# cschin/Peregrine

Hardware: AMD Instinct MI355X
Metric: confirmed overlaps/sec (ovlp_t records, index+overlap stages, seqdb resident in HBM) (higher is better)
Workload: dtype u8/u32 integer

## Files before the change

### peregrine_amd/csrc/pgx_replay.h

```cpp
#pragma once
#include "pgx_internal.h"

namespace pgx {
namespace rp {

constexpr uint32_t NIL = 0;
constexpr uint32_t NONE = 0xFFFFFFFFu;
constexpr int END_FUZZ = 48;
enum { T_OVERLAP = 0, T_CONTAINS = 1, T_CONTAINED = 2 };

constexpr uint32_t NIN = 58;
struct alignas(16) PHot {
  unsigned long long key;
  uint32_t own;
  uint32_t pad;
};
struct alignas(256) PCold {
  uint32_t cnt;
  uint32_t rhead;
  uint32_t in[NIN];
  uint32_t pad[4];
};
static_assert(sizeof(PHot) == 16 && sizeof(PCold) == 256, "pair slot = 16 hot bytes + four cold cache lines");
struct MSlot {
  unsigned long long a;
  uint32_t b;
  uint32_t req;
};
struct Item {
  uint32_t pslot;
  uint32_t info;
  uint32_t mslot;
  uint32_t next;
};
struct RNode {
  uint32_t next, bucket;
};
constexpr uint32_t I_GUESS = 1u << 18, I_UNFILED = 1u << 19;
#ifndef PGX_SPARSE_CAP
#define PGX_SPARSE_CAP 65536
#endif
constexpr uint32_t SPARSE_CAP = PGX_SPARSE_CAP;
constexpr uint32_t LIST_CAP = 262144;
constexpr uint32_t DEV_LIST = 0xFFFFFFFFu, DEV_LIST_WIN = 0xFFFFFFFEu;
enum : uint32_t { OV_ITEMS = 1, OV_NODES = 2, OV_REQS = 4, OV_PAIRS = 8, OV_MEMO = 16, OV_QOFF = 32, OV_PASSES = 64 };
constexpr uint8_t F_DUP = 1, F_GUESS = 2, F_UNFILED = 4;
constexpr uint8_t F_BIG = 8;

struct alignas(64) Counters {
  uint32_t item_top, rnode_top, nreq, overflow;
  uint32_t pad0[12];
  uint32_t ndirty, min_dirty, max_dirty, pad;
  uint32_t nbig;
  uint32_t nbig_total;
  uint32_t pad1[10];
  unsigned long long lookups, skips, evals, records;
#ifdef PGX_BIG_STATS
  uint32_t big_max_steps, big_long, big_long_n, big_evals;
  unsigned long long big_pairs, pad2[1];
#else
  unsigned long long pad2[4];
#endif
};

struct R {
  uint32_t nb;
  const uint32_t *bid, *bstart;
  const uint64_t *y0;
  const uint8_t *dir;
  const uint32_t *rlen;
  PHot *ph;
  PCold *pc;
  uint32_t cshift;
  uint32_t pmask;
  MSlot *mt;
  uint32_t mmask;
  Item *items;
  uint32_t item_cap;
  RNode *rn;
  uint32_t rn_cap;
  pgx_align_key *rq_key;
  pgx_match *rq_res;
  uint32_t req_cap, settled;
  uint32_t memo_used;
  uint8_t *dirty, *evaluated, *parity, *bflags, *ever;
  uint32_t *ihead, *inum, *ohead, *lookups, *skips;
  uint32_t *dlist;
  uint32_t *blist;
  uint32_t wlist0;
  uint4 *wcur;
  Counters *c;
  unsigned long long *spread;
// ... 113 lines not shown
  const uint32_t *w = reinterpret_cast<const uint32_t *>(&r.pc[slot >> r.cshift]);
  const uint4 h1 = *reinterpret_cast<const uint4 *>(w);
  const uint32_t c = min(h1.x, NIN);
  if (c > 0 && h1.z > j + 1 && h1.z <= r.nb) r.dirty[h1.z - 1] = 1;
  if (c > 1 && h1.w > j + 1 && h1.w <= r.nb) r.dirty[h1.w - 1] = 1;
  for (uint32_t q = 2; q < c; q += 8) {
    const uint4 a = *reinterpret_cast<const uint4 *>(w + 2 + q), b = *reinterpret_cast<const uint4 *>(w + 6 + q);
    const uint32_t x[8] = {a.x, a.y, a.z, a.w, b.x, b.y, b.z, b.w};
#pragma unroll
    for (uint32_t k = 0; k < 8; ++k)
      if (q + k < c && x[k] > j + 1 && x[k] <= r.nb) r.dirty[x[k] - 1] = 1;
  }
  if (c < NIN) return;
  for (uint32_t nd = h1.y; nd != NIL; nd = r.rn[nd - 1].next) {
    const uint32_t rb = r.rn[nd - 1].bucket;
    if (rb > j) r.dirty[rb] = 1;
  }
}

struct M128 {
  uint64_t lo, hi;
};
__device__ __forceinline__ int popc128(M128 m) { return __popcll(m.lo) + __popcll(m.hi); }
__device__ __forceinline__ bool any128(M128 m) { return (m.lo | m.hi) != 0; }
__device__ __forceinline__ int ctz128(M128 m) { return m.lo ? __builtin_ctzll(m.lo) : 64 + __builtin_ctzll(m.hi); }
__device__ __forceinline__ int nth128(M128 m, uint32_t nth) {
  const uint32_t cl = (uint32_t)__popcll(m.lo);
  uint64_t w = m.lo;
  int base = 0;
  if (nth > cl) w = m.hi, nth -= cl, base = 64;
  for (uint32_t k = 1; k < nth; ++k) w &= w - 1;
  return base + __builtin_ctzll(w);
}
__device__ __forceinline__ M128 upto128(int stop) {
  M128 m;
  m.lo = stop >= 63 ? ~0ULL : ((2ULL << stop) - 1ULL);
  m.hi = stop < 64 ? 0ULL : (stop >= 127 ? ~0ULL : ((2ULL << (stop - 64)) - 1ULL));
  return m;
}
__device__ __forceinline__ M128 and128(M128 a, M128 b) { return M128{a.lo & b.lo, a.hi & b.hi}; }
__device__ __forceinline__ M128 andn128(M128 a, M128 b) { return M128{a.lo & ~b.lo, a.hi & ~b.hi}; }
__device__ __forceinline__ M128 shr128(M128 m, uint32_t s) {
  if (s >= 128) return M128{0, 0};
  if (s >= 64) return M128{m.hi >> (s - 64), 0};
  if (s == 0) return m;
  return M128{m.lo >> s | m.hi << (64 - s), m.hi >> s};
}
__device__ __forceinline__ M128 shl128(M128 m, uint32_t s) {
  if (s >= 128) return M128{0, 0};
  if (s >= 64) return M128{0, m.lo << (s - 64)};
  if (s == 0) return m;
  return M128{m.lo << s, m.hi << s | m.lo >> (64 - s)};
}
__device__ __forceinline__ M128 or128(M128 a, M128 b) { return M128{a.lo | b.lo, a.hi | b.hi}; }




constexpr int LOOK_NB = 4;
constexpr uint8_t FACT_VALID = 1, FACT_PRESENT = 2, FACT_ACCEPTED = 4, FACT_GUESSED = 8, FACT_UNFILED = 16;
constexpr int FACT_TYPE_SHIFT = 5;
#ifndef PGX_BIG_NW
#define PGX_BIG_NW 8
#endif
constexpr int BIG_NW = PGX_BIG_NW;
constexpr int BIG_NR = BIG_NW / 2;
constexpr uint32_t BIG_WG = 512;
constexpr uint32_t SET_CAP = 2048, CLAIM_CAP = 1024;
constexpr uint32_t CB = 4096;

__global__ void k_setup(R r, uint32_t *hist);
__global__ void k_init_slots(uint4 *__restrict__ wcur, uint32_t nslots, uint32_t n_dense, uint32_t wlist0, Counters *c);
__global__ void k_eval(R r, uint32_t lo, uint32_t hi, uint32_t nlist);
template <int GLT, int PW>
__global__ void k_eval_rows(R r, uint32_t lo, uint32_t hi, uint32_t nlist);
__global__ void k_eval_big(R r, uint32_t lo, uint32_t hi, uint32_t nlist);
__global__ void k_update(R r, uint32_t lo, uint32_t hi, uint32_t nlist);
__global__ void k_count_a(R r, uint32_t rlo, uint32_t rhi, uint32_t *__restrict__ blk);
__global__ void k_count_b(R r, uint32_t rlo, uint32_t rhi, const uint32_t *__restrict__ blk, uint32_t nblk);
__global__ void k_file(R r, uint32_t limit);
__global__ void k_settle(R r);
__global__ void k_emit(R r, const uint32_t *__restrict__ off, pgx_ovlp *__restrict__ out);
__global__ void k_count_pairs(const PHot *__restrict__ ph, uint32_t cap, unsigned long long *__restrict__ out);

}
}
```

### peregrine_amd/csrc/pgx_replay.hip

```cpp
#include <optional>

#include "pgx_replay.h"

namespace pgx {
using namespace rp;
namespace {
uint32_t pow2_at_least(size_t x) {
  size_t c = 1024;
  while (c < x) c <<= 1;
  return (uint32_t)c;
}
unsigned cdiv256(size_t n) { return (unsigned)((n + 255) / 256); }
int env_int(const char *name, int unset) { return getenv(name) ? atoi(getenv(name)) : unset; }
template <typename T>
void alloc_tagged(const char *tag, DevBuf<T> &buf, size_t n) { MemTag t(tag); buf.alloc(n); }

constexpr size_t ITEMS_PER_ENTRY = 6, ITEMS_PER_BUCKET = 64, NODES_PER_ENTRY = 8, REQS_PER_ENTRY = 1;
constexpr size_t STATE_PER_BUCKET = 64;
constexpr double TABLE_LOAD = 0.4;

struct Usage {
  double pairs = 0, reqs = 0, items = 0, nodes = 0;
  void raise(const Usage &u) { pairs = std::max(pairs, u.pairs), reqs = std::max(reqs, u.reqs), items = std::max(items, u.items), nodes = std::max(nodes, u.nodes); }
};
// ... 199 lines not shown
    if (r.big_min || r.dup_min) {
      fetch(false);
      use_big = hc->nbig_total != 0;
    }
    cblk.alloc((nb + CB - 1) / CB * 3);
  }
  void setup_with_histogram() {
    DevBuf<uint32_t> hist(32);
    PGX_HIP(hipMemsetAsync(hist.p, 0, 32 * sizeof(uint32_t), s));
    hipLaunchKernelGGL(k_setup, dim3(cdiv256(nb)), dim3(256), 0, s, r, hist.p);
    uint32_t h[32];
    hist.download(h, 32);
    sync();
    fprintf(stderr, "[pgx]   buckets by entries / 8 (last class: >= 120):");
    for (int i = 0; i < 16; ++i) fprintf(stderr, " %u", h[i]);
    fprintf(stderr, "\n[pgx]   ... of those holding a read twice (one partner at a time):");
    for (int i = 0; i < 16; ++i) fprintf(stderr, " %u", h[16 + i]);
    fprintf(stderr, "\n");
  }
  void fetch(bool totals, bool counters = true) {
    if (counters) PGX_HIP(hipMemcpyAsync(hc, dc.p, sizeof(Counters), hipMemcpyDeviceToHost, s));
    if (totals) PGX_HIP(hipMemcpyAsync(rs.hs, spread.p, SPREAD * 8 * sizeof(unsigned long long), hipMemcpyDeviceToHost, s));
    sync();
    if (totals) sum_totals();
  }
  void sum_totals() {
    const unsigned long long *hs = rs.hs;
    hc->evals = hc->lookups = hc->skips = 0;
    hc->records = 0;
    for (uint32_t i = 0; i < SPREAD; ++i) hc->evals += hs[i * 8], hc->lookups += hs[i * 8 + 1], hc->skips += hs[i * 8 + 2], hc->records += hs[i * 8 + 7];
#ifdef PGX_BIG_STATS
    unsigned long long b3 = 0, b4 = 0, b5 = 0, b6 = 0, b7 = 0;
    for (uint32_t i = 0; i < SPREAD; ++i) b3 += hs[i * 8 + 3], b4 += hs[i * 8 + 4], b5 += hs[i * 8 + 5], b6 += hs[i * 8 + 6], b7 += hs[i * 8 + 7];
    fprintf(stderr, "[pgx]   k_eval_big so far: %u evaluations, %llu steps, %llu rows committed; steps cut at a duplicate %llu, ended by a containment %llu, all rows %llu; longest %u steps, %u evaluations of >= 64 steps (entries %u); %llu pairs looked up\n",
            hc->big_evals, b3, b4, b5, b6, b7, hc->big_max_steps, hc->big_long, hc->big_long_n, hc->big_pairs);
#endif
#ifdef PGX_SETTLE_STATS
    unsigned long long c3 = 0, c4 = 0, c5 = 0, c6 = 0;
    for (uint32_t i = 0; i < SPREAD; ++i) c3 += hs[i * 8 + 3], c4 += hs[i * 8 + 4], c5 += hs[i * 8 + 5], c6 += hs[i * 8 + 6];
    fprintf(stderr, "[pgx]   wrong guesses so far: type %llu, rejected short overlap %llu, rejected no match %llu, rejected other %llu\n", c3, c4, c5, c6);
#endif
  }
  void learn_dirty() { n_dirty = hc->ndirty, known = true, d_lo = n_dirty ? hc->min_dirty : 0, d_hi = n_dirty ? hc->max_dirty + 1 : 0; }
  uint32_t gave_up(uint32_t ov) {
    if (trace || !(ov & (OV_ITEMS | OV_NODES | OV_REQS | OV_PAIRS | OV_MEMO)))
      fprintf(stderr, "[pgx] note: the device replay gave up (code %u: items %u of %u, reader nodes %u of %u, requests %u of %u)\n", ov,
              hc->item_top, r.item_cap, hc->rnode_top, r.rn_cap, hc->nreq, r.req_cap);
    return ov;
  }
  void count(uint32_t lo = 0, uint32_t hi = NONE) {
    hi = std::min<uint32_t>(hi, (uint32_t)nb);
    const uint32_t nbl = std::max<uint32_t>(1, (hi - lo + CB - 1) / CB);
    std::optional<KernelTimer> tm;
    if (timed) tm.emplace("replay_misc", 0);
    hipLaunchKernelGGL(k_count_a, dim3(nbl), dim3(256), 0, s, r, lo, hi, cblk.p);
    hipLaunchKernelGGL(k_count_b, dim3(nbl), dim3(256), 0, s, r, lo, hi, cblk.p, nbl);
  }
  void count_all() { count(), have_list = true; }
  void pass(uint32_t lo, uint32_t hi, uint32_t list, Narrow narrow, uint32_t groups, uint64_t units) {
    std::optional<KernelTimer> tm;
    if (timed) tm.emplace(narrow == Narrow::rows ? "replay_rows" : "replay_dense", units);
    const bool walled = deep && list != DEV_LIST;
    double td = 0, t_eval = 0;
    if (walled) sync(), td = wall_ms();
    if (list == DEV_LIST_WIN) count(lo, hi);
    const uint32_t a = list ? 0u : lo, b = list ? (uint32_t)nb : hi;
    const uint32_t big_a = list == DEV_LIST_WIN ? LIST_CAP : list == DEV_LIST ? groups : lo;
    const dim3 big_grid(std::min<uint32_t>(BIG_WG, groups)), big_block(64 * BIG_NW), grid(cdiv256((size_t)groups * GL));
// ... 266 lines not shown
```

### peregrine_amd/csrc/pgx_replay_eval.hip

```cpp
#include "pgx_replay.h"

namespace pgx {
namespace rp {

__global__ __launch_bounds__(256) void k_eval(R r, uint32_t lo, uint32_t hi, uint32_t nlist) {
  __shared__ uint32_t s_rid[GPB][128], s_pos[GPB][128], s_rl[GPB][128];
  __shared__ uint8_t s_dir[GPB][128];
  const int lane = threadIdx.x & 63, gl = lane & (GL - 1), gbase = lane & ~(GL - 1), gib = threadIdx.x / GL;
  const uint32_t wave = (blockIdx.x * blockDim.x + threadIdx.x) >> 6;
  const uint64_t jj = bucket_of_group(r, lo, hi, nlist, wave * GPW + (uint32_t)(lane / GL));
  const uint32_t j = (uint32_t)jj;
  bool alive = jj < hi && r.dirty[j] && !r.c->overflow;
  if (alive && (r.bflags[j] & F_BIG)) {
    if (gl == 0) {
      const uint32_t at = atomicAdd(&r.c->nbig, 1u);
      if (at < LIST_CAP) r.blist[at] = j;
    }
    alive = false;
  }
  {
    const uint64_t am = __ballot(alive);
    if (!am) return;
    if (lane == (int)__builtin_ctzll(am)) atomicAdd(&r.spread[(wave % SPREAD) * 8], (unsigned long long)(__popcll(am) / GL));
  }
// ... 471 lines not shown
          if ((uint64_t)base + take > r.item_cap) {
            atomicOr(&r.c->overflow, OV_ITEMS);
            return;
          }
          icur = base, iend = base + take;
        }
        fresh = icur, icur += want;
      }
      auto base_of = [&](uint32_t no) { return no >= first_new ? fresh + 16u * (no - first_new) : chunk; };
      if (my_ins) {
        const uint32_t ord = num + (uint32_t)__popcll(ins & ((1ULL << gl) - 1ULL));
        const uint32_t idx = base_of(ord >> 4) + (ord & 15);
        uint32_t next;
        if (ord == 0) next = NIL;
        else if ((ord & 15) == 0) next = base_of((ord >> 4) - 1) + 16;
        else next = idx;
        uint32_t info = (uint32_t)myrow | pi << 8 | type << 16;
        if (guessed) info |= I_GUESS;
        if (mslot == NONE) info |= I_UNFILED;
        r.items[idx] = Item{slot, info, mslot, next};
      }
      chunk = base_of(last_no);
      head = chunk + (last & 15) + 1;
      num += cins;
    }
    {
      const uint64_t g1 = gbits(__ballot(my_ins && guessed), gbase), g2 = gbits(__ballot(my_ins && mslot == NONE), gbase);
      any_guess |= g1 != 0, any_unfiled |= g2 != 0;
    }
  }
}
template __global__ void k_eval_rows<64, 16>(R r, uint32_t lo, uint32_t hi, uint32_t nlist);

__global__ __launch_bounds__(64 * BIG_NW) void k_eval_big(R r, uint32_t lo, uint32_t hi, uint32_t nlist) {
  enum { MV = 0, MP, MPO, MA, MAO, MAC, MAP, MGU, MUF, MDF, NM };
  __shared__ uint32_t s_rid[128], s_pos[128], s_rl[128];
  __shared__ uint8_t s_dir[128];
  __shared__ uint64_t s_m[BIG_NW][NM];
  __shared__ uint32_t s_fresh, s_abort, s_bail;
  __shared__ unsigned long long s_setk[SET_CAP];
  __shared__ uint8_t s_sett[SET_CAP];
  __shared__ unsigned long long s_clk[CLAIM_CAP];
  __shared__ uint32_t s_clw[CLAIM_CAP];
  __shared__ uint8_t s_fact[128 * 128];
  __shared__ M128 s_vis[128], s_ins[128];
  __shared__ uint32_t s_rbase[128], s_wsum[2];
  const int lane = threadIdx.x & 63, w = threadIdx.x >> 6;
  const uint32_t wave_id = r.wbig0 + blockIdx.x * BIG_NW + (uint32_t)w;
  const uint4 wc = r.wcur[wave_id];
  uint32_t rcur = wc.x, rend = wc.y;
  uint32_t icur = wc.z, iend = wc.w;
  if (threadIdx.x == 0) s_abort = 0;
  const uint32_t list_limit = nlist ? lo : 0u;
  const uint32_t nbig = min(r.c->nbig, LIST_CAP);
  for (uint32_t g = blockIdx.x; g < nbig; g += gridDim.x) {
  {
    const uint32_t e = r.blist[g];
    if ((e & 0x80000000u) && (e & 0x7FFFFFFFu) >= list_limit) continue;
    const uint32_t j = (e & 0x80000000u) ? (r.dlist[e & 0x7FFFFFFFu] & 0x7FFFFFFFu) : e;
    __syncthreads();
    if (threadIdx.x == 0) {
      if (r.c->overflow) s_abort = 1;
      s_bail = 0, s_fresh = (j < hi && r.dirty[j]) ? 1u : 0u;
    }
    __syncthreads();
    if (s_abort) break;
    if (!s_fresh) continue;
    const uint32_t b = r.bid[j], s0 = r.bstart[b], n = r.bstart[b + 1] - s0;
    const bool first_eval = r.ever[j] == 0;
    const bool dup = (r.bflags[j] & F_DUP) != 0;
    for (uint32_t i = threadIdx.x; i < n; i += blockDim.x) {
      const uint64_t y = r.y0[s0 + i];
      const uint32_t rid = (uint32_t)(y >> 32);
      s_rid[i] = rid, s_pos[i] = (((uint32_t)y) >> 1) + 1, s_dir[i] = r.dir[s0 + i], s_rl[i] = r.rlen[rid];
    }
    if (threadIdx.x < 128) s_vis[threadIdx.x] = M128{0, 0}, s_ins[threadIdx.x] = M128{0, 0};
    if (dup) {
      for (uint32_t i = threadIdx.x; i < SET_CAP; i += blockDim.x) s_setk[i] = 0;
      for (uint32_t i = threadIdx.x; i < CLAIM_CAP; i += blockDim.x) s_clk[i] = 0, s_clw[i] = 0xFFFFFFFFu;
    }
    __syncthreads();
    if (threadIdx.x == 0) {
      r.dirty[j] = 0, r.evaluated[j] = 1, r.ever[j] = 1, r.parity[j] ^= 1, r.ohead[j] = r.ihead[j];
      atomicAdd(&r.spread[(blockIdx.x % SPREAD) * 8], 1ULL);
    }
#ifdef PGX_BIG_STATS
    uint32_t st_steps = 0, st_rows = 0, st_cut = 0, st_cont = 0, st_full = 0, st_pairs = 0;
#endif
    {
      const uint32_t total = (n >> 1) * n;
      for (uint32_t base = 0; base < total; base += LOOK_NB * blockDim.x) {
        uint32_t row[LOOK_NB], par[LOOK_NB], at[LOOK_NB], own[LOOK_NB];
        unsigned long long pair[LOOK_NB];
        bool inb[LOOK_NB], live[LOOK_NB];
#pragma unroll
        for (int k = 0; k < LOOK_NB; ++k) {
          const uint32_t idx = base + (uint32_t)k * blockDim.x + threadIdx.x;
          const uint32_t f = idx / n, c = idx - f * n;
          inb[k] = idx < total;
          if (c < n - 1 - f) row[k] = f, par[k] = f + 1 + c;
          else row[k] = n - 2 - f, par[k] = c, inb[k] = inb[k] && row[k] != f;
          uint32_t rid0 = 0, rid1 = 0;
          if (inb[k]) rid0 = s_rid[row[k]], rid1 = s_rid[par[k]];
          live[k] = inb[k] && rid0 != rid1;
          pair[k] = rid0 < rid1 ? ((unsigned long long)rid0 << 32 | rid1) : ((unsigned long long)rid1 << 32 | rid0);
          at[k] = (uint32_t)mix64(pair[k]) & r.pmask, own[k] = 0;
        }
        uint8_t fact[LOOK_NB];
        bool absent[LOOK_NB];
#pragma unroll
        for (int k = 0; k < LOOK_NB; ++k) fact[k] = live[k] ? FACT_VALID : 0, absent[k] = live[k];
#ifdef PGX_BIG_STATS
#pragma unroll
        for (int k = 0; k < LOOK_NB; ++k) st_pairs += live[k] ? 1u : 0u;
#endif
        for (int probes = 0; probes < 1024; ++probes) {
          uint4 h[LOOK_NB];
#pragma unroll
          for (int k = 0; k < LOOK_NB; ++k) h[k] = *reinterpret_cast<const uint4 *>(&r.ph[at[k]]);
          bool more = false;
// ... 35 lines not shown
#pragma unroll
            for (int k = 0; k < LOOK_NB; ++k) {
              if (!live[k]) continue;
              const unsigned long long cur = (unsigned long long)h[k].y << 32 | h[k].x;
              if (cur == 0) live[k] = false;
              else if (cur == ma[k] && h[k].z == mb[k] + 1) req[k] = h[k].w, unfiled[k] = false, live[k] = false;
              else at[k] = (at[k] + 1) & r.mmask, more = true;
            }
            if (!more) break;
          }
        }
        pgx_match res[LOOK_NB];
#pragma unroll
        for (int k = 0; k < LOOK_NB; ++k)
          if (absent[k] && req[k] < r.settled) res[k] = r.rq_res[req[k]];
#pragma unroll
        for (int k = 0; k < LOOK_NB; ++k) {
          if (absent[k]) {
            bool accepted, guessed = false;
            uint32_t type;
            if (req[k] < r.settled) {
              accepted = classify(res[k], rlen0[k], rlen1[k], q_off[k], &type);
            } else {
              accepted = true, guessed = true, type = T_OVERLAP;
              if (r.predict && predict_contained(rlen0[k], rlen1[k], q_off[k], r.predict, r.predict2)) type = rlen0[k] >= rlen1[k] ? T_CONTAINS : T_CONTAINED;
            }
            fact[k] |= (uint8_t)((accepted ? FACT_ACCEPTED : 0) | (guessed ? FACT_GUESSED : 0) | (unfiled[k] ? FACT_UNFILED : 0) | type << FACT_TYPE_SHIFT);
          }
          if (inb[k]) s_fact[row[k] * 128 + par[k]] = fact[k];
        }
      }
    }
    __syncthreads();
    uint64_t clo = 0, chi = 0;
    auto cget = [&](uint32_t i) { return (((i < 64 ? clo : chi) >> (i & 63)) & 1) != 0; };
    auto cset = [&](uint32_t i) {
      if (i < 64) clo |= 1ULL << i;
      else chi |= 1ULL << (i - 64);
    };
    uint32_t head = NIL, num = 0, lookups = 0, skips = 0;
    bool any_guess = false, any_unfiled = false;
    int done_to = (int)n - 1;
    bool row_open = false;
    int cur_row = 0;
    uint32_t pbase = 0, got = 0;
    for (;;) {
      int a[BIG_NR], nrows = 0;
#pragma unroll
      for (int k = 0; k < BIG_NR; ++k) a[k] = -1;
      if (row_open) {
        a[0] = cur_row, nrows = 1;
      } else {
        int x = done_to;
#pragma unroll
        for (int k = 0; k < BIG_NR; ++k) {
          if (x >= 0) {
            do --x;
            while (x >= 0 && cget((uint32_t)x));
          }
          if (x >= 0) a[k] = x, nrows = k + 1;
        }
      }
      if (nrows == 0 || r.bestn == 0) break;
      const int q = w >> 1, off = (w & 1) * 64 + lane;
      int myrow = -1;
#pragma unroll
      for (int k = 0; k < BIG_NR; ++k)
        if (k == q) myrow = a[k];
      const uint32_t first = row_open ? pbase : (uint32_t)(myrow + 1);
      const uint32_t pi = first + (uint32_t)off;
      const uint32_t wi = (uint32_t)(q * 128 + off);
      bool valid = q < nrows && pi < n && !cget(pi);
      uint32_t fact = 0;
      unsigned long long pair = 0;
      if (valid) {
        fact = s_fact[myrow * 128 + (int)pi];
        const uint32_t rid0 = s_rid[myrow], rid1 = s_rid[pi];
        pair = rid0 < rid1 ? ((unsigned long long)rid0 << 32 | rid1) : ((unsigned long long)rid1 << 32 | rid0);
        valid = (fact & FACT_VALID) != 0;
      }
      bool present = false, accepted = false, guessed = false, unfiled = true;
      uint32_t ptype = 0, type = 0;
      if (valid) {
        present = (fact & FACT_PRESENT) != 0;
        ptype = present ? fact >> FACT_TYPE_SHIFT : 0;
        if (!present && dup) {
          for (uint32_t i = (uint32_t)mix64(pair) & (SET_CAP - 1);; i = (i + 1) & (SET_CAP - 1)) {
            const unsigned long long kk = s_setk[i];
            if (kk == 0) break;
            if (kk == pair + 1) {
              present = true, ptype = s_sett[i];
              break;
            }
          }
        }
        if (!present) accepted = (fact & FACT_ACCEPTED) != 0, guessed = (fact & FACT_GUESSED) != 0, unfiled = (fact & FACT_UNFILED) != 0, type = fact >> FACT_TYPE_SHIFT;
      }
      const bool ins0 = valid && !present && accepted;
      uint32_t my_claim = NONE;
      if (dup) {
        if (ins0) {
          for (uint32_t i = (uint32_t)(mix64(pair) >> 20) & (CLAIM_CAP - 1);; i = (i + 1) & (CLAIM_CAP - 1)) {
            unsigned long long kk = s_clk[i];
            if (kk == 0) kk = atomicCAS(&s_clk[i], 0ULL, (unsigned long long)pair + 1), kk = kk ? kk : pair + 1;
            if (kk == pair + 1) {
              atomicMin(&s_clw[i], wi);
              my_claim = i;
              break;
            }
          }
        }
      }
      {
        const uint64_t mv = __ballot(valid), mp = __ballot(valid && present), mpo = __ballot(valid && present && ptype == T_OVERLAP);
        const uint64_t ma = __ballot(ins0), mao = __ballot(ins0 && type == T_OVERLAP), mac = __ballot(ins0 && type == T_CONTAINED);
        const uint64_t map = __ballot(ins0 && type == T_CONTAINS), mgu = __ballot(ins0 && guessed), muf = __ballot(ins0 && unfiled);
        if (lane == 0)
          s_m[w][MV] = mv, s_m[w][MP] = mp, s_m[w][MPO] = mpo, s_m[w][MA] = ma, s_m[w][MAO] = mao, s_m[w][MAC] = mac, s_m[w][MAP] = map,
          s_m[w][MGU] = mgu, s_m[w][MUF] = muf, s_m[w][MDF] = 0;
      }
      __syncthreads();
      if (dup) {
        bool dflag = false;
        if (my_claim != NONE) {
          dflag = s_clw[my_claim] < wi;
        } else if (valid && !present) {
          for (uint32_t i = (uint32_t)(mix64(pair) >> 20) & (CLAIM_CAP - 1);; i = (i + 1) & (CLAIM_CAP - 1)) {
            const unsigned long long kk = s_clk[i];
            if (kk == 0) break;
            if (kk == pair + 1) {
              dflag = s_clw[i] < wi;
              break;
            }
          }
        }
        const uint64_t mdf = __ballot(dflag);
        if (lane == 0) s_m[w][MDF] = mdf;
        __syncthreads();
      }
      M128 proc[BIG_NR];
#pragma unroll
      for (int k = 0; k < BIG_NR; ++k) proc[k] = M128{0, 0};
      int committed = 0;
      bool open_next = false;
      int open_row = 0;
      uint32_t open_pbase = 0, open_got = 0;
#pragma unroll
      for (int k = 0; k < BIG_NR; ++k) {
        if (k >= nrows) break;
        const uint32_t first_k = row_open ? pbase : (uint32_t)(a[k] + 1);
        const M128 gone = shr128(M128{clo, chi}, first_k);
        const M128 inc = andn128(M128{s_m[2 * k][MPO] | s_m[2 * k][MAO], s_m[2 * k + 1][MPO] | s_m[2 * k + 1][MAO]}, gone);
        const M128 ac = andn128(M128{s_m[2 * k][MAC], s_m[2 * k + 1][MAC]}, gone), ap = andn128(M128{s_m[2 * k][MAP], s_m[2 * k + 1][MAP]}, gone);
        const M128 df = andn128(M128{s_m[2 * k][MDF], s_m[2 * k + 1][MDF]}, gone);
        const int cut = any128(df) ? ctz128(df) : 128;
        if (cut == 0) break;
        const uint32_t need = r.bestn - (row_open ? got : 0u);
        int stop = 128;
        if ((uint32_t)popc128(inc) >= need) stop = nth128(inc, need);
        if (any128(ac)) stop = min(stop, ctz128(ac));
        const bool complete = stop < cut || (cut == 128);
        proc[k] = andn128(complete ? upto128(stop) : upto128(cut - 1), gone);
        const M128 apk = and128(ap, proc[k]);
        for (uint64_t m = apk.lo; m; m &= m - 1) cset(first_k + (uint32_t)__builtin_ctzll(m));
        for (uint64_t m = apk.hi; m; m &= m - 1) cset(first_k + 64u + (uint32_t)__builtin_ctzll(m));
        const bool rowc = any128(and128(ac, proc[k]));
        if (rowc) cset((uint32_t)a[k]);
        if (!complete) {
          open_next = true, open_row = a[k], open_pbase = first_k + (uint32_t)cut, open_got = (row_open ? got : 0u) + (uint32_t)popc128(and128(inc, proc[k]));
          break;
        }
        ++committed;
      }
#ifdef PGX_BIG_STATS
      ++st_steps, st_rows += (uint32_t)committed, st_cut += open_next ? 1u : 0u, st_full += (committed == nrows) ? 1u : 0u;
      st_cont += (!open_next && committed < nrows) ? 1u : 0u;
#endif
#pragma unroll
      for (int k = 0; k < BIG_NR; ++k)
        if ((int)threadIdx.x == k && k < nrows && any128(proc[k])) {
          const uint32_t first_k = row_open ? pbase : (uint32_t)(a[k] + 1);
          const M128 v = shl128(and128(M128{s_m[2 * k][MV], s_m[2 * k + 1][MV]}, proc[k]), first_k);
          const M128 in = shl128(and128(M128{s_m[2 * k][MA], s_m[2 * k + 1][MA]}, proc[k]), first_k);
          s_vis[a[k]] = or128(s_vis[a[k]], v), s_ins[a[k]] = or128(s_ins[a[k]], in);
        }
#pragma unroll
      for (int k = 0; k < BIG_NR; ++k)
        if (k == committed - 1) done_to = a[k];
      row_open = open_next;
      if (open_next) cur_row = open_row, pbase = open_pbase, got = open_got;
      uint64_t myproc = 0;
#pragma unroll
      for (int ww = 0; ww < BIG_NW; ++ww) {
        const int k = ww >> 1;
        const uint64_t pw = (ww & 1) ? proc[k].hi : proc[k].lo;
        if (ww == w) myproc = pw;
        num += (uint32_t)__popcll(s_m[ww][MA] & pw);
        skips += (uint32_t)__popcll(s_m[ww][MP] & pw);
        lookups += (uint32_t)__popcll(s_m[ww][MV] & ~s_m[ww][MP] & pw);
        any_guess |= (s_m[ww][MGU] & pw) != 0, any_unfiled |= (s_m[ww][MUF] & pw) != 0;
      }
      if (dup) {
        const bool my_ins = ins0 && ((myproc >> lane) & 1);
        if (my_claim != NONE) s_clk[my_claim] = 0, s_clw[my_claim] = 0xFFFFFFFFu;
        if (my_ins) {
          uint32_t tries = 0;
          for (uint32_t i = (uint32_t)mix64(pair) & (SET_CAP - 1);; i = (i + 1) & (SET_CAP - 1)) {
            const unsigned long long kk = atomicCAS(&s_setk[i], 0ULL, (unsigned long long)pair + 1);
            if (kk == 0 || kk == pair + 1) {
              s_sett[i] = (uint8_t)type;
              break;
            }
            if (++tries >= SET_CAP) {
              s_bail = 1;
              break;
            }
          }
        }
      }
      __syncthreads();
      if (s_bail) break;
    }
    bool p_reg = false;
    uint32_t p_idx = 0, p_slot = 0;
    auto resolve_pending = [&]() {
      if (p_reg && p_idx < NIN) r.pc[p_slot >> r.cshift].in[p_idx] = j + 1, p_reg = false;
      const uint64_t rm = __ballot(p_reg);
      if (rm) {
        const uint32_t total = (uint32_t)__popcll(rm);
        if (rcur + total > rend) {
          uint32_t base = 0;
          if (lane == 0) base = atomicAdd(&r.c->rnode_top, NCH);
          base = (uint32_t)__shfl((int)base, 0, 64);
          if ((uint64_t)base + NCH > r.rn_cap) {
            atomicOr(&r.c->overflow, OV_NODES);
            s_abort = 1;
            p_reg = false;
            return;
          }
          rcur = base, rend = base + NCH;
        }
        if (p_reg) {
          const uint32_t node = rcur + lane_rank(rm);
          const uint32_t old = atomicExch(&r.pc[p_slot >> r.cshift].rhead, node + 1);
          r.rn[node] = RNode{old, j};
        }
        rcur += total;
        p_reg = false;
      }
    };
    if (!s_bail) {
      if (threadIdx.x < 128) {
        const int row = (int)n - 2 - (int)threadIdx.x;
        const uint32_t c = row >= 0 ? (uint32_t)popc128(s_ins[row]) : 0u;
        uint32_t incl = c;
// ... 41 lines not shown
            const uint4 h1 = *reinterpret_cast<const uint4 *>(pw);
            const uint32_t c = min(h1.x, NIN);
            if ((c > 0 && h1.z == j + 1) || (c > 1 && h1.w == j + 1)) reg = false;
            for (uint32_t qq = 2; qq < c && reg; qq += 8) {
              const uint4 xa = *reinterpret_cast<const uint4 *>(pw + 2 + qq), xb = *reinterpret_cast<const uint4 *>(pw + 6 + qq);
              const uint32_t x[8] = {xa.x, xa.y, xa.z, xa.w, xb.x, xb.y, xb.z, xb.w};
#pragma unroll
              for (uint32_t k = 0; k < 8; ++k)
                if (qq + k < c && x[k] == j + 1) reg = false;
            }
          }
          if (reg) p_idx = atomicAdd(&r.pc[slot >> r.cshift].cnt, 1u), p_slot = slot, p_reg = true;
          if (my_ins) {
            const uint32_t ord = s_rbase[row] + ((int)n - 2 - row >= 64 ? s_wsum[0] : 0u) + (half ? (uint32_t)__popcll(s_ins[row].lo) : 0u) +
                                 (uint32_t)__popcll(im & ((1ULL << lane) - 1ULL));
            const uint32_t idx = fresh + ord;
            uint32_t info = (uint32_t)row | pi << 8 | (fact >> FACT_TYPE_SHIFT) << 16;
            if (fact & FACT_GUESSED) info |= I_GUESS;
            if (mslot == NONE) info |= I_UNFILED;
            r.items[idx] = Item{slot, info, mslot, ord == 0 ? NIL : idx};
          }
        }
        if (num) head = fresh + num;
      }
    }
    resolve_pending();
#ifdef PGX_BIG_STATS
    {
      for (int o = 32; o; o >>= 1) st_pairs += (uint32_t)__shfl_xor((int)st_pairs, o, 64);
      if (lane == 0) atomicAdd(&r.c->big_pairs, (unsigned long long)st_pairs);
    }
    if (threadIdx.x == 0) {
      unsigned long long *line = r.spread + (blockIdx.x % SPREAD) * 8;
      atomicAdd(line + 3, (unsigned long long)st_steps), atomicAdd(line + 4, (unsigned long long)st_rows), atomicAdd(line + 5, (unsigned long long)st_cut);
      atomicAdd(line + 6, (unsigned long long)st_cont), atomicAdd(line + 7, (unsigned long long)st_full);
      atomicMax(&r.c->big_max_steps, st_steps);
      if (st_steps >= 64) atomicAdd(&r.c->big_long, 1u), atomicAdd(&r.c->big_long_n, n);
      atomicAdd(&r.c->big_evals, 1u);
    }
#endif
    if (threadIdx.x == 0) {
      if (s_bail) {
        r.dirty[j] = 1, r.evaluated[j] = 0, r.parity[j] ^= 1;
        r.bflags[j] = (uint8_t)((r.bflags[j] & ~F_BIG));
      } else {
        r.ihead[j] = head, r.inum[j] = num, r.lookups[j] = lookups, r.skips[j] = skips;
        r.bflags[j] = (uint8_t)(F_BIG | (dup ? F_DUP : 0) | (any_guess ? F_GUESS : 0) | (any_unfiled ? F_UNFILED : 0));
      }
    }
  }
  if (s_abort) break;
  }
  if (lane == 0) r.wcur[wave_id] = make_uint4(rcur, rend, icur, iend);
}

}
}
```

Before: 64.40 million.

## Run big-entry walk in a single wave without block barriers

Replaces the multi-wave walk in k_eval_big with a walk done by wave 0 alone. It processes one row at a time, 64 partners per pass, using ballots in registers in place of shared-memory mask exchange and __syncthreads per step. Duplicate detection now uses a precomputed same-read chain (s_same) in place of the shared claim hash table, which frees shared memory. The trade is less parallelism across rows and waves during the walk, while block-wide barriers and claim atomics go away. Optional phase timing stats are also added.

New measurement: 65.76 million (median of 6 runs). +2.1%, better.

```diff
diff --git a/peregrine_amd/csrc/pgx_replay.h b/peregrine_amd/csrc/pgx_replay.h
--- a/peregrine_amd/csrc/pgx_replay.h
+++ b/peregrine_amd/csrc/pgx_replay.h
@@ -56,8 +56,10 @@
   uint32_t pad1[10];
   unsigned long long lookups, skips, evals, records;
 #ifdef PGX_BIG_STATS
-  uint32_t big_max_steps, big_long, big_long_n, big_evals;
+  uint32_t big_max_passes, big_long, big_long_n, big_evals;
   unsigned long long big_pairs, pad2[1];
+  unsigned long long big_cyc[3], big_lmax, big_cyc_long[3];
+  uint32_t big_ticket, big_launches;
 #else
   unsigned long long pad2[4];
 #endif
@@ -237,6 +239,10 @@
   for (uint32_t k = 1; k < nth; ++k) w &= w - 1;
   return base + __builtin_ctzll(w);
 }
+__device__ __forceinline__ int nth64(uint64_t m, uint32_t nth) {
+  for (uint32_t k = 1; k < nth; ++k) m &= m - 1;
+  return __builtin_ctzll(m);
+}
 __device__ __forceinline__ M128 upto128(int stop) {
   M128 m;
   m.lo = stop >= 63 ? ~0ULL : ((2ULL << stop) - 1ULL);
@@ -271,7 +277,7 @@
 constexpr int BIG_NW = PGX_BIG_NW;
 constexpr int BIG_NR = BIG_NW / 2;
 constexpr uint32_t BIG_WG = 512;
-constexpr uint32_t SET_CAP = 2048, CLAIM_CAP = 1024;
+constexpr uint32_t SET_CAP = 2048;
 constexpr uint32_t CB = 4096;
 
 __global__ void k_setup(R r, uint32_t *hist);
diff --git a/peregrine_amd/csrc/pgx_replay.hip b/peregrine_amd/csrc/pgx_replay.hip
--- a/peregrine_amd/csrc/pgx_replay.hip
+++ b/peregrine_amd/csrc/pgx_replay.hip
@@ -255,8 +255,15 @@
 #ifdef PGX_BIG_STATS
     unsigned long long b3 = 0, b4 = 0, b5 = 0, b6 = 0, b7 = 0;
     for (uint32_t i = 0; i < SPREAD; ++i) b3 += hs[i * 8 + 3], b4 += hs[i * 8 + 4], b5 += hs[i * 8 + 5], b6 += hs[i * 8 + 6], b7 += hs[i * 8 + 7];
-    fprintf(stderr, "[pgx]   k_eval_big so far: %u evaluations, %llu steps, %llu rows committed; steps cut at a duplicate %llu, ended by a containment %llu, all rows %llu; longest %u steps, %u evaluations of >= 64 steps (entries %u); %llu pairs looked up\n",
-            hc->big_evals, b3, b4, b5, b6, b7, hc->big_max_steps, hc->big_long, hc->big_long_n, hc->big_pairs);
+    fprintf(stderr, "[pgx]   k_eval_big so far: %u evaluations, %llu row passes, %llu rows committed; passes cut at a duplicate %llu, rows ended by a containment %llu, rows of more than one pass %llu; longest %u passes, %u evaluations of >= 64 passes (entries %u); %llu pairs looked up\n",
+            hc->big_evals, b3, b4, b5, b6, b7, hc->big_max_passes, hc->big_long, hc->big_long_n, hc->big_pairs);
+    {
+      const unsigned long long *a = hc->big_cyc, *l = hc->big_cyc_long;
+      const double sa = (double)(a[0] + a[1] + a[2]), sl = (double)(l[0] + l[1] + l[2]);
+      fprintf(stderr, "[pgx]   k_eval_big phases, all evaluations: LOOK %.2f ms, WALK %.2f, COMMIT %.2f (%.0f / %.0f / %.0f %%); the longest evaluation of each of %u launches: LOOK %.2f ms, WALK %.2f, COMMIT %.2f (%.0f / %.0f / %.0f %%)\n",
+              a[0] * 1e-5, a[1] * 1e-5, a[2] * 1e-5, sa ? 100 * a[0] / sa : 0, sa ? 100 * a[1] / sa : 0, sa ? 100 * a[2] / sa : 0, hc->big_launches,
+              l[0] * 1e-5, l[1] * 1e-5, l[2] * 1e-5, sl ? 100 * l[0] / sl : 0, sl ? 100 * l[1] / sl : 0, sl ? 100 * l[2] / sl : 0);
+    }
 #endif
 #ifdef PGX_SETTLE_STATS
     unsigned long long c3 = 0, c4 = 0, c5 = 0, c6 = 0;
diff --git a/peregrine_amd/csrc/pgx_replay_eval.hip b/peregrine_amd/csrc/pgx_replay_eval.hip
--- a/peregrine_amd/csrc/pgx_replay_eval.hip
+++ b/peregrine_amd/csrc/pgx_replay_eval.hip
@@ -527,16 +527,15 @@
 }
 template __global__ void k_eval_rows<64, 16>(R r, uint32_t lo, uint32_t hi, uint32_t nlist);
 
+#define BIG_WAVE_SYNC() __builtin_amdgcn_fence(__ATOMIC_RELEASE, "wavefront"), __builtin_amdgcn_fence(__ATOMIC_ACQUIRE, "wavefront")
 __global__ __launch_bounds__(64 * BIG_NW) void k_eval_big(R r, uint32_t lo, uint32_t hi, uint32_t nlist) {
-  enum { MV = 0, MP, MPO, MA, MAO, MAC, MAP, MGU, MUF, MDF, NM };
   __shared__ uint32_t s_rid[128], s_pos[128], s_rl[128];
   __shared__ uint8_t s_dir[128];
-  __shared__ uint64_t s_m[BIG_NW][NM];
   __shared__ uint32_t s_fresh, s_abort, s_bail;
+  __shared__ uint32_t s_walk[4];
   __shared__ unsigned long long s_setk[SET_CAP];
   __shared__ uint8_t s_sett[SET_CAP];
-  __shared__ unsigned long long s_clk[CLAIM_CAP];
-  __shared__ uint32_t s_clw[CLAIM_CAP];
+  __shared__ uint16_t s_same[128];
   __shared__ uint8_t s_fact[128 * 128];
   __shared__ M128 s_vis[128], s_ins[128];
   __shared__ uint32_t s_rbase[128], s_wsum[2];
@@ -572,15 +571,28 @@
     if (threadIdx.x < 128) s_vis[threadIdx.x] = M128{0, 0}, s_ins[threadIdx.x] = M128{0, 0};
     if (dup) {
       for (uint32_t i = threadIdx.x; i < SET_CAP; i += blockDim.x) s_setk[i] = 0;
-      for (uint32_t i = threadIdx.x; i < CLAIM_CAP; i += blockDim.x) s_clk[i] = 0, s_clw[i] = 0xFFFFFFFFu;
     }
     __syncthreads();
+    if (dup) {
+      for (uint32_t i = threadIdx.x; i < n; i += blockDim.x) {
+        const uint32_t me = s_rid[i];
+        uint32_t prev = 0, more = 0;
+        for (uint32_t k = 0; k < n; ++k) {
+          const bool same = s_rid[k] == me && k != i;
+          more |= same ? 0x100u : 0u;
+          if (same && k < i) prev = k + 1;
+        }
+        s_same[i] = (uint16_t)(prev | more);
+      }
+    }
     if (threadIdx.x == 0) {
       r.dirty[j] = 0, r.evaluated[j] = 1, r.ever[j] = 1, r.parity[j] ^= 1, r.ohead[j] = r.ihead[j];
       atomicAdd(&r.spread[(blockIdx.x % SPREAD) * 8], 1ULL);
     }
 #ifdef PGX_BIG_STATS
-    uint32_t st_steps = 0, st_rows = 0, st_cut = 0, st_cont = 0, st_full = 0, st_pairs = 0;
+    uint32_t st_passes = 0, st_rows = 0, st_cut = 0, st_cont = 0, st_multi = 0, st_pairs = 0;
+    unsigned long long st_t0 = 0, st_t1 = 0, st_t2 = 0;
+    if (threadIdx.x == 0) st_t0 = wall_clock64();
 #endif
     {
       const uint32_t total = (n >> 1) * n;
@@ -682,195 +694,141 @@
       }
     }
     __syncthreads();
-    uint64_t clo = 0, chi = 0;
-    auto cget = [&](uint32_t i) { return (((i < 64 ? clo : chi) >> (i & 63)) & 1) != 0; };
-    auto cset = [&](uint32_t i) {
-      if (i < 64) clo |= 1ULL << i;
-      else chi |= 1ULL << (i - 64);
-    };
-    uint32_t head = NIL, num = 0, lookups = 0, skips = 0;
-    bool any_guess = false, any_unfiled = false;
-    int done_to = (int)n - 1;
-    bool row_open = false;
-    int cur_row = 0;
-    uint32_t pbase = 0, got = 0;
-    for (;;) {
-      int a[BIG_NR], nrows = 0;
-#pragma unroll
-      for (int k = 0; k < BIG_NR; ++k) a[k] = -1;
-      if (row_open) {
-        a[0] = cur_row, nrows = 1;
-      } else {
-        int x = done_to;
-#pragma unroll
-        for (int k = 0; k < BIG_NR; ++k) {
-          if (x >= 0) {
-            do --x;
-            while (x >= 0 && cget((uint32_t)x));
-          }
-          if (x >= 0) a[k] = x, nrows = k + 1;
-        }
-      }
-      if (nrows == 0 || r.bestn == 0) break;
-      const int q = w >> 1, off = (w & 1) * 64 + lane;
-      int myrow = -1;
-#pragma unroll
-      for (int k = 0; k < BIG_NR; ++k)
-        if (k == q) myrow = a[k];
-      const uint32_t first = row_open ? pbase : (uint32_t)(myrow + 1);
-      const uint32_t pi = first + (uint32_t)off;
-      const uint32_t wi = (uint32_t)(q * 128 + off);
-      bool valid = q < nrows && pi < n && !cget(pi);
-      uint32_t fact = 0;
-      unsigned long long pair = 0;
-      if (valid) {
-        fact = s_fact[myrow * 128 + (int)pi];
-        const uint32_t rid0 = s_rid[myrow], rid1 = s_rid[pi];
-        pair = rid0 < rid1 ? ((unsigned long long)rid0 << 32 | rid1) : ((unsigned long long)rid1 << 32 | rid0);
-        valid = (fact & FACT_VALID) != 0;
-      }
-      bool present = false, accepted = false, guessed = false, unfiled = true;
-      uint32_t ptype = 0, type = 0;
-      if (valid) {
-        present = (fact & FACT_PRESENT) != 0;
-        ptype = present ? fact >> FACT_TYPE_SHIFT : 0;
-        if (!present && dup) {
-          for (uint32_t i = (uint32_t)mix64(pair) & (SET_CAP - 1);; i = (i + 1) & (SET_CAP - 1)) {
-            const unsigned long long kk = s_setk[i];
-            if (kk == 0) break;
-            if (kk == pair + 1) {
-              present = true, ptype = s_sett[i];
-              break;
+#ifdef PGX_BIG_STATS
+    if (threadIdx.x == 0) st_t1 = wall_clock64();
+#endif
+    if (__builtin_amdgcn_readfirstlane(w) == 0) {
+      __builtin_amdgcn_s_setprio(3);
+      uint64_t clo = 0, chi = 0;
+      uint32_t num = 0, lookups = 0, skips = 0;
+      bool any_guess = false, any_unfiled = false, bail = false;
+      uint32_t set_n = 0;
+      int row = (int)n - 1;
+      while (r.bestn != 0 && !bail) {
+        {
+          const M128 below{row >= 64 ? ~0ULL : (1ULL << row) - 1ULL, row > 64 ? (1ULL << (row - 64)) - 1ULL : 0ULL};
+          const M128 open = andn128(below, M128{clo, chi});
+          if (!any128(open)) break;
+          row = open.hi ? 127 - __builtin_clzll(open.hi) : 63 - __builtin_clzll(open.lo);
+        }
+        uint32_t first = (uint32_t)row + 1, got = 0;
+        M128 vis{0, 0}, ins{0, 0};
+        const uint32_t row_twice = dup ? (uint32_t)__builtin_amdgcn_readfirstlane((int)s_same[row]) & 0x100u : 0u;
+#ifdef PGX_BIG_STATS
+        uint32_t row_passes = 0;
+#endif
+        for (;;) {
+          const uint32_t pi = first + (uint32_t)lane;
+          const uint64_t gone = first < 64 ? clo >> first | (chi << 1) << (63 - first) : chi >> (first - 64);
+          uint32_t fact = 0, same = 0;
+          if (pi < n) {
+            fact = s_fact[row * 128 + (int)pi];
+            if (dup) same = s_same[pi];
+          }
+          const bool twice = pi < n && ((row_twice | same) & 0x100u) != 0;
+          unsigned long long pair = 0;
+          if (twice) {
+            const uint32_t rid0 = s_rid[row], rid1 = s_rid[pi];
+            pair = rid0 < rid1 ? ((unsigned long long)rid0 << 32 | rid1) : ((unsigned long long)rid1 << 32 | rid0);
+          }
+          if (set_n) {
+            if (twice && (fact & (FACT_VALID | FACT_PRESENT)) == FACT_VALID) {
+              for (uint32_t i = (uint32_t)mix64(pair) & (SET_CAP - 1);; i = (i + 1) & (SET_CAP - 1)) {
+                const unsigned long long kk = s_setk[i];
+                if (kk == 0) break;
+                if (kk == pair + 1) {
+                  fact = FACT_VALID | FACT_PRESENT | (uint32_t)s_sett[i] << FACT_TYPE_SHIFT;
+                  break;
+                }
+              }
             }
           }
-        }
-        if (!present) accepted = (fact & FACT_ACCEPTED) != 0, guessed = (fact & FACT_GUESSED) != 0, unfiled = (fact & FACT_UNFILED) != 0, type = fact >> FACT_TYPE_SHIFT;
-      }
-      const bool ins0 = valid && !present && accepted;
-      uint32_t my_claim = NONE;
-      if (dup) {
-        if (ins0) {
-          for (uint32_t i = (uint32_t)(mix64(pair) >> 20) & (CLAIM_CAP - 1);; i = (i + 1) & (CLAIM_CAP - 1)) {
-            unsigned long long kk = s_clk[i];
-            if (kk == 0) kk = atomicCAS(&s_clk[i], 0ULL, (unsigned long long)pair + 1), kk = kk ? kk : pair + 1;
-            if (kk == pair + 1) {
-              atomicMin(&s_clw[i], wi);
-              my_claim = i;
-              break;
+          const uint32_t ty = fact >> FACT_TYPE_SHIFT;
+          const uint64_t mv = __ballot((fact & FACT_VALID) != 0) & ~gone;
+          const uint64_t mp = __ballot((fact & FACT_PRESENT) != 0) & mv;
+          const uint64_t ma = __ballot((fact & FACT_ACCEPTED) != 0) & mv & ~mp;
+          const uint64_t mto = __ballot(ty == T_OVERLAP), mtc = __ballot(ty == T_CONTAINED), mtp = __ballot(ty == T_CONTAINS);
+          const uint64_t mgu = __ballot((fact & FACT_GUESSED) != 0), muf = __ballot((fact & FACT_UNFILED) != 0);
+          const uint64_t inc = (mp | ma) & mto;
+          const uint64_t ac = ma & mtc;
+          const uint64_t ap = ma & mtp;
+          uint64_t df = 0;
+          const uint64_t absent = mv & ~mp;
+          if (dup && ma && (absent & (absent - 1))) {
+            bool dflag = false;
+            if ((absent >> lane) & 1) {
+              for (uint32_t p = same & 0xFFu; p > first; p = s_same[p - 1] & 0xFFu)
+                if ((ma >> (p - 1 - first)) & 1) {
+                  dflag = true;
+                  break;
+                }
             }
-          }
-        }
-      }
-      {
-        const uint64_t mv = __ballot(valid), mp = __ballot(valid && present), mpo = __ballot(valid && present && ptype == T_OVERLAP);
-        const uint64_t ma = __ballot(ins0), mao = __ballot(ins0 && type == T_OVERLAP), mac = __ballot(ins0 && type == T_CONTAINED);
-        const uint64_t map = __ballot(ins0 && type == T_CONTAINS), mgu = __ballot(ins0 && guessed), muf = __ballot(ins0 && unfiled);
-        if (lane == 0)
-          s_m[w][MV] = mv, s_m[w][MP] = mp, s_m[w][MPO] = mpo, s_m[w][MA] = ma, s_m[w][MAO] = mao, s_m[w][MAC] = mac, s_m[w][MAP] = map,
-          s_m[w][MGU] = mgu, s_m[w][MUF] = muf, s_m[w][MDF] = 0;
-      }
-      __syncthreads();
-      if (dup) {
-        bool dflag = false;
-        if (my_claim != NONE) {
-          dflag = s_clw[my_claim] < wi;
-        } else if (valid && !present) {
-          for (uint32_t i = (uint32_t)(mix64(pair) >> 20) & (CLAIM_CAP - 1);; i = (i + 1) & (CLAIM_CAP - 1)) {
-            const unsigned long long kk = s_clk[i];
-            if (kk == 0) break;
-            if (kk == pair + 1) {
-              dflag = s_clw[i] < wi;
-              break;
+            df = __ballot(dflag);
+          }
+          const int cut = df ? (int)__builtin_ctzll(df) : 64;
+          const uint32_t need = r.bestn - got;
+          int stop = 64;
+          if ((uint32_t)__popcll(inc) >= need) stop = nth64(inc, need);
+          if (ac) stop = min(stop, (int)__builtin_ctzll(ac));
+          const bool ends = stop < cut;
+          const int last = ends ? stop : cut - 1;
+          const uint64_t proc = last >= 63 ? ~0ULL : (2ULL << last) - 1ULL;
+          const uint64_t pv = mv & proc, pins = ma & proc, apk = ap & proc;
+          num += (uint32_t)__popcll(pins), skips += (uint32_t)__popcll(mp & proc), lookups += (uint32_t)__popcll(pv & ~mp);
+          got += (uint32_t)__popcll(inc & proc);
+          any_guess |= (mgu & pins) != 0, any_unfiled |= (muf & pins) != 0;
+          auto up = [&](uint64_t m) { return first < 64 ? M128{m << first, (m >> 1) >> (63 - first)} : M128{0, m << (first - 64)}; };
+          vis = or128(vis, up(pv)), ins = or128(ins, up(pins));
+          {
+            const M128 c = up(apk);
+            clo |= c.lo, chi |= c.hi;
+          }
+          if (ac & proc) {
+            if (row < 64) clo |= 1ULL << row;
+            else chi |= 1ULL << (row - 64);
+          }
+#ifdef PGX_BIG_STATS
+          ++st_passes, ++row_passes, st_cut += (!ends && cut < 64) ? 1u : 0u, st_cont += (ac & proc) ? 1u : 0u;
+#endif
+          const uint64_t pset = __ballot(twice) & pins;
+          if (pset) {
+            bool full = false;
+            set_n += (uint32_t)__popcll(pset);
+            if ((pset >> lane) & 1) {
+              uint32_t tries = 0;
+              for (uint32_t i = (uint32_t)mix64(pair) & (SET_CAP - 1);; i = (i + 1) & (SET_CAP - 1)) {
+                const unsigned long long kk = atomicCAS(&s_setk[i], 0ULL, (unsigned long long)pair + 1);
+                if (kk == 0 || kk == pair + 1) {
+                  s_sett[i] = (uint8_t)ty;
+                  break;
+                }
+                if (++tries >= SET_CAP) {
+                  full = true;
+                  break;
+                }
+              }
             }
-          }
-        }
-        const uint64_t mdf = __ballot(dflag);
-        if (lane == 0) s_m[w][MDF] = mdf;
-        __syncthreads();
-      }
-      M128 proc[BIG_NR];
-#pragma unroll
-      for (int k = 0; k < BIG_NR; ++k) proc[k] = M128{0, 0};
-      int committed = 0;
-      bool open_next = false;
-      int open_row = 0;
-      uint32_t open_pbase = 0, open_got = 0;
-#pragma unroll
-      for (int k = 0; k < BIG_NR; ++k) {
-        if (k >= nrows) break;
-        const uint32_t first_k = row_open ? pbase : (uint32_t)(a[k] + 1);
-        const M128 gone = shr128(M128{clo, chi}, first_k);
-        const M128 inc = andn128(M128{s_m[2 * k][MPO] | s_m[2 * k][MAO], s_m[2 * k + 1][MPO] | s_m[2 * k + 1][MAO]}, gone);
-        const M128 ac = andn128(M128{s_m[2 * k][MAC], s_m[2 * k + 1][MAC]}, gone), ap = andn128(M128{s_m[2 * k][MAP], s_m[2 * k + 1][MAP]}, gone);
-        const M128 df = andn128(M128{s_m[2 * k][MDF], s_m[2 * k + 1][MDF]}, gone);
-        const int cut = any128(df) ? ctz128(df) : 128;
-        if (cut == 0) break;
-        const uint32_t need = r.bestn - (row_open ? got : 0u);
-        int stop = 128;
-        if ((uint32_t)popc128(inc) >= need) stop = nth128(inc, need);
-        if (any128(ac)) stop = min(stop, ctz128(ac));
-        const bool complete = stop < cut || (cut == 128);
-        proc[k] = andn128(complete ? upto128(stop) : upto128(cut - 1), gone);
-        const M128 apk = and128(ap, proc[k]);
-        for (uint64_t m = apk.lo; m; m &= m - 1) cset(first_k + (uint32_t)__builtin_ctzll(m));
-        for (uint64_t m = apk.hi; m; m &= m - 1) cset(first_k + 64u + (uint32_t)__builtin_ctzll(m));
-        const bool rowc = any128(and128(ac, proc[k]));
-        if (rowc) cset((uint32_t)a[k]);
-        if (!complete) {
-          open_next = true, open_row = a[k], open_pbase = first_k + (uint32_t)cut, open_got = (row_open ? got : 0u) + (uint32_t)popc128(and128(inc, proc[k]));
-          break;
-        }
-        ++committed;
-      }
+            BIG_WAVE_SYNC();
+            bail = __ballot(full) != 0;
+          }
+          first += (uint32_t)(cut < 64 ? cut : 64);
+          if (ends || bail || first >= n) break;
+        }
+        if (lane == 0 && any128(vis)) s_vis[row] = vis, s_ins[row] = ins;
 #ifdef PGX_BIG_STATS
-      ++st_steps, st_rows += (uint32_t)committed, st_cut += open_next ? 1u : 0u, st_full += (committed == nrows) ? 1u : 0u;
-      st_cont += (!open_next && committed < nrows) ? 1u : 0u;
+        ++st_rows, st_multi += row_passes > 1 ? 1u : 0u;
 #endif
-#pragma unroll
-      for (int k = 0; k < BIG_NR; ++k)
-        if ((int)threadIdx.x == k && k < nrows && any128(proc[k])) {
-          const uint32_t first_k = row_open ? pbase : (uint32_t)(a[k] + 1);
-          const M128 v = shl128(and128(M128{s_m[2 * k][MV], s_m[2 * k + 1][MV]}, proc[k]), first_k);
-          const M128 in = shl128(and128(M128{s_m[2 * k][MA], s_m[2 * k + 1][MA]}, proc[k]), first_k);
-          s_vis[a[k]] = or128(s_vis[a[k]], v), s_ins[a[k]] = or128(s_ins[a[k]], in);
-        }
-#pragma unroll
-      for (int k = 0; k < BIG_NR; ++k)
-        if (k == committed - 1) done_to = a[k];
-      row_open = open_next;
-      if (open_next) cur_row = open_row, pbase = open_pbase, got = open_got;
-      uint64_t myproc = 0;
-#pragma unroll
-      for (int ww = 0; ww < BIG_NW; ++ww) {
-        const int k = ww >> 1;
-        const uint64_t pw = (ww & 1) ? proc[k].hi : proc[k].lo;
-        if (ww == w) myproc = pw;
-        num += (uint32_t)__popcll(s_m[ww][MA] & pw);
-        skips += (uint32_t)__popcll(s_m[ww][MP] & pw);
-        lookups += (uint32_t)__popcll(s_m[ww][MV] & ~s_m[ww][MP] & pw);
-        any_guess |= (s_m[ww][MGU] & pw) != 0, any_unfiled |= (s_m[ww][MUF] & pw) != 0;
-      }
-      if (dup) {
-        const bool my_ins = ins0 && ((myproc >> lane) & 1);
-        if (my_claim != NONE) s_clk[my_claim] = 0, s_clw[my_claim] = 0xFFFFFFFFu;
-        if (my_ins) {
-          uint32_t tries = 0;
-          for (uint32_t i = (uint32_t)mix64(pair) & (SET_CAP - 1);; i = (i + 1) & (SET_CAP - 1)) {
-            const unsigned long long kk = atomicCAS(&s_setk[i], 0ULL, (unsigned long long)pair + 1);
-            if (kk == 0 || kk == pair + 1) {
-              s_sett[i] = (uint8_t)type;
-              break;
-            }
-            if (++tries >= SET_CAP) {
-              s_bail = 1;
-              break;
-            }
-          }
-        }
-      }
-      __syncthreads();
-      if (s_bail) break;
-    }
+      }
+      __builtin_amdgcn_s_setprio(0);
+      if (lane == 0) s_walk[0] = num, s_walk[1] = lookups, s_walk[2] = skips, s_walk[3] = (any_guess ? 1u : 0u) | (any_unfiled ? 2u : 0u), s_bail = bail ? 1u : 0u;
+    }
+    __syncthreads();
+    const uint32_t num = s_walk[0], lookups = s_walk[1], skips = s_walk[2];
+    const bool any_guess = (s_walk[3] & 1) != 0, any_unfiled = (s_walk[3] & 2) != 0;
+    uint32_t head = NIL;
+#ifdef PGX_BIG_STATS
+    if (threadIdx.x == 0) st_t2 = wall_clock64();
+#endif
     bool p_reg = false;
     uint32_t p_idx = 0, p_slot = 0;
     auto resolve_pending = [&]() {
@@ -978,11 +936,14 @@
     }
     if (threadIdx.x == 0) {
       unsigned long long *line = r.spread + (blockIdx.x % SPREAD) * 8;
-      atomicAdd(line + 3, (unsigned long long)st_steps), atomicAdd(line + 4, (unsigned long long)st_rows), atomicAdd(line + 5, (unsigned long long)st_cut);
-      atomicAdd(line + 6, (unsigned long long)st_cont), atomicAdd(line + 7, (unsigned long long)st_full);
-      atomicMax(&r.c->big_max_steps, st_steps);
-      if (st_steps >= 64) atomicAdd(&r.c->big_long, 1u), atomicAdd(&r.c->big_long_n, n);
+      atomicAdd(line + 3, (unsigned long long)st_passes), atomicAdd(line + 4, (unsigned long long)st_rows), atomicAdd(line + 5, (unsigned long long)st_cut);
+      atomicAdd(line + 6, (unsigned long long)st_cont), atomicAdd(line + 7, (unsigned long long)st_multi);
+      atomicMax(&r.c->big_max_passes, st_passes);
+      if (st_passes >= 64) atomicAdd(&r.c->big_long, 1u), atomicAdd(&r.c->big_long_n, n);
       atomicAdd(&r.c->big_evals, 1u);
+      const unsigned long long t3 = wall_clock64(), tl = st_t1 - st_t0, tw = st_t2 - st_t1, tc = t3 - st_t2;
+      atomicAdd(&r.c->big_cyc[0], tl), atomicAdd(&r.c->big_cyc[1], tw), atomicAdd(&r.c->big_cyc[2], tc);
+      atomicMax(&r.c->big_lmax, (t3 - st_t0) << 40 | (tw & 0xFFFFF) << 20 | (tl & 0xFFFFF));
     }
 #endif
     if (threadIdx.x == 0) {
@@ -998,7 +959,21 @@
   if (s_abort) break;
   }
   if (lane == 0) r.wcur[wave_id] = make_uint4(rcur, rend, icur, iend);
+#ifdef PGX_BIG_STATS
+  if (threadIdx.x == 0) {
+    __threadfence();
+    if (atomicAdd(&r.c->big_ticket, 1u) == gridDim.x - 1) {
+      const unsigned long long m = atomicExch(&r.c->big_lmax, 0ULL);
+      if (m) {
+        const unsigned long long tl = m & 0xFFFFF, tw = (m >> 20) & 0xFFFFF;
+        r.c->big_cyc_long[0] += tl, r.c->big_cyc_long[1] += tw, r.c->big_cyc_long[2] += (m >> 40) - tl - tw, r.c->big_launches += 1;
+      }
+      r.c->big_ticket = 0;
+    }
+  }
+#endif
 }
+#undef BIG_WAVE_SYNC
 
 }
 }
```
